# lhn0323/BEVFUSION-3D_object_detection

Hardware: AMD Instinct MI355X
Metric: nuScenes frames/sec (6-cam+LiDAR BEVFusion fwd+bwd) (higher is better)
Workload: dtype bf16; 1 GPU; full: BEVFusion camera+LiDAR (ResNet-50, LSS 6x256x704, hard voxelize 40k pts, sparse encoder, ConvFuser, SECOND/SECONDFPN, TransFusion head + Hungarian targets + focal/L1/gaussian-focal losses) fwd + bwd + clip + AdamW, bf16 autocast, fp32 index paths; global_batch=4, points_per_frame=40000, parallelism=independent frames per rank, execution=eager launches on 2 HIP queues (camera / BEV chain, LiDAR branch), view_transform_conv_dtype=bf16, head_fp32_conv=three bf16 products per multiply, fp32 accumulation (2^-16 relative per product), dense_weight_gradients=one grouped launch per tile shape at the end of the backward pass, backward_pass_thread=caller, trainable_params=37361053

## Files before the change

### bevfusion-3d_object_detection_amd/_lib.py

```python
import ctypes
import os

import torch

_HERE = os.path.dirname(os.path.abspath(__file__))
LIB_PATH = os.path.join(_HERE, "csrc", "libbevfusion_hip.so")

_c_int = ctypes.c_int
_c_vp = ctypes.c_void_p
_c_sz = ctypes.c_size_t

SIGNATURES = {
    "bfhip_abi_version": (_c_int, []),
    "bfhip_last_error": (ctypes.c_char_p, []),
    "bfhip_profile_enable": (None, [_c_int]),
    "bfhip_profile_read": (_c_int, [_c_int, _c_vp, _c_vp, _c_int]),
    "bfhip_bev_pool_fwd": (_c_int, [_c_vp] * 5 + [_c_int] * 7 + [_c_vp, _c_vp]),
    "bfhip_bev_pool_bwd": (_c_int, [_c_vp] * 5 + [_c_int] * 8 + [_c_vp, _c_vp]),
    "bfhip_dynamic_voxelize": (_c_int, [_c_vp, _c_vp, _c_int, _c_int, _c_vp, _c_vp, _c_vp]),
    "bfhip_hard_voxelize_workspace_bytes": (_c_sz, [_c_int, _c_int, _c_int]),
    "bfhip_hard_voxelize": (_c_int, [_c_vp, _c_int, _c_int, _c_vp, _c_vp, _c_vp, _c_vp, _c_vp,
                                     _c_int, _c_int, _c_vp, _c_sz, _c_vp, _c_vp]),
    "bfhip_bev_plan_workspace_bytes": (_c_sz, [ctypes.c_longlong, ctypes.c_longlong]),
    "bfhip_bev_plan": (_c_int, [_c_vp] * 7 + [_c_int] * 4 + [_c_vp] * 3 + [_c_vp] * 11 + [_c_int, _c_vp, _c_sz, _c_vp]),
# ... 77 lines not shown
    "bfhip_conv2d_dgrad_wt": (_c_int, [_c_vp, _c_int, _c_vp, _c_vp, _c_int, _c_vp, _c_int] + [_c_int] * 11 + [_c_vp]),
    "bfhip_conv2d_dgrad_fuses_addend": (_c_int, [_c_int] * 5),
    "bfhip_split_bf16x3": (_c_int, [_c_vp, ctypes.c_longlong, _c_int, _c_vp, _c_int, _c_vp, _c_int, _c_vp]),
    "bfhip_conv2d_wt_segment_bytes": (_c_int, []),
    "bfhip_conv2d_weight_transpose_batched": (_c_int, [_c_vp, _c_int, ctypes.c_longlong, _c_vp]),
    "bfhip_conv2d_launch_choice": (_c_int, [_c_int] * 12 + [_c_vp]),
    "bfhip_conv2d_wgrad_choice": (_c_int, [_c_int] * 10 + [_c_vp]),
    "bfhip_conv2d_wgrad_workspace_bytes": (_c_sz, [_c_int] * 7),
    "bfhip_conv2d_wgrad": (_c_int, [_c_vp, _c_int, _c_vp, _c_int, _c_vp] + [_c_int] * 11 + [_c_vp, _c_sz, _c_vp]),
    "bfhip_conv2d_wgrad_group_table_bytes": (_c_sz, [_c_int]),
    "bfhip_conv2d_wgrad_groupable": (_c_int, [_c_int] * 10),
    "bfhip_conv2d_wgrad_group_plan": (_c_int, [_c_vp, _c_int, _c_int, _c_vp, _c_sz, _c_vp]),
    "bfhip_conv2d_wgrad_group_launch": (_c_int, [_c_vp, _c_vp, _c_vp, _c_sz, _c_vp]),
    "bfhip_bn2d_fwd_partials": (_c_int, [_c_vp] * 4 + [ctypes.c_longlong, _c_int, _c_int, ctypes.c_float, ctypes.c_float, _c_int] +
                                [_c_vp] * 4 + [_c_vp, _c_int, _c_vp, _c_vp]),
    "bfhip_bn2d_fwd_partials_mask": (_c_int, [_c_vp] * 4 + [ctypes.c_longlong, _c_int, _c_int, ctypes.c_float, ctypes.c_float, _c_int] +
                                     [_c_vp] * 4 + [_c_vp, _c_int, _c_vp, _c_vp, _c_vp]),
    "bfhip_bn2d_bwd_mask": (_c_int, [_c_vp] * 5 + [ctypes.c_longlong, _c_int, _c_int] + [_c_vp] * 4 + [_c_vp, _c_sz, _c_vp]),
    "bfhip_adamw_segment_bytes": (_c_int, []),
    "bfhip_adamw_chunk_elems": (_c_int, []),
    "bfhip_adamw_step": (_c_int, [_c_vp, _c_vp, _c_vp, _c_int, _c_vp, _c_vp] + [ctypes.c_float] * 6 + [_c_vp]),
    "bfhip_query_losses": (_c_int, [_c_vp] * 7 + [_c_int] * 6 + [ctypes.c_float, ctypes.c_float] + [_c_vp] * 4),
    "bfhip_swin_attn_supported": (_c_int, [_c_int] * 7),
    "bfhip_swin_attn_parts": (_c_int, [_c_int] * 4),
    "bfhip_swin_attn_fwd": (_c_int, [_c_vp, ctypes.c_longlong, _c_vp] + [_c_int] * 5 + [ctypes.c_float, _c_vp, _c_vp, _c_vp]),
    "bfhip_swin_attn_bwd": (_c_int, [_c_vp, ctypes.c_longlong, _c_vp, _c_vp, _c_vp, _c_vp] + [_c_int] * 5 +
                            [ctypes.c_float, _c_vp, _c_vp, _c_int, _c_vp]),
    "bfhip_layernorm_supported": (_c_int, [ctypes.c_longlong, _c_int, _c_int, _c_int]),
    "bfhip_layernorm_parts": (_c_int, [ctypes.c_longlong, _c_int]),
    "bfhip_layernorm_fwd": (_c_int, [_c_vp, _c_vp, _c_vp, ctypes.c_longlong, _c_vp, _c_vp, ctypes.c_longlong, _c_int, ctypes.c_float] +
                            [_c_int] * 3 + [_c_vp] * 4),
    "bfhip_layernorm_bwd": (_c_int, [_c_vp] * 6 + [ctypes.c_longlong, ctypes.c_longlong] + [_c_int] * 4 + [_c_vp] * 3 + [_c_int] +
                            [_c_vp] * 3),
}

_lib = None


def load():
    global _lib
    if _lib is None:
        if not os.path.exists(LIB_PATH):
            raise RuntimeError(
                "libbevfusion_hip.so not found at %s: build it with "
                "`python -c 'import __graft_entry__ as g; g.build()'` (hipcc, gfx950). "
                "There is no CPU fallback." % LIB_PATH)
        lib = ctypes.CDLL(LIB_PATH)
        for name, (res, args) in SIGNATURES.items():
            fn = getattr(lib, name)
            fn.restype = res
            fn.argtypes = args
        _lib = lib
    return _lib


_torch_ext = False


def torch_ext():
    global _torch_ext
    if _torch_ext is False:
        _torch_ext = None
        path = os.path.join(_HERE, "csrc", "bfhip_torch_ext.so")
        if os.environ.get("BFHIP_TORCH_EXT", "1") == "1" and os.path.exists(path):
            import importlib.util
            load()
# ... 33 lines not shown

def ptr(t):
    return None if t is None else t.data_ptr()


_raw_stream = getattr(torch._C, "_cuda_getCurrentRawStream", None)


def stream_of(t):
    if _raw_stream is not None:
        return _raw_stream(t.device.index if t.device.index is not None else torch.cuda.current_device())
    return ctypes.c_void_p(torch.cuda.current_stream(t.device).cuda_stream)


def host_i32(values):
    return (ctypes.c_int32 * len(values))(*[int(v) for v in values])


def host_f32(values):
    arr = (ctypes.c_float * len(values))(*[float(v) for v in values])
    return arr


def require_cuda(t, name):
    if not t.is_cuda:
        raise RuntimeError("%s must be a CUDA(HIP) tensor; this build has no CPU path" % name)
    if not t.is_contiguous():
        raise RuntimeError("%s must be contiguous" % name)


OPS = dict(bev_pool_fwd=0, bev_pool_bwd=1, hard_voxelize=2, dynamic_voxelize=3, lift_splat_fwd=4, lift_splat_bwd=5,
           spconv_fwd=6, spconv_bwd=7, rulebook=8, bev_aux=9, scatter_fwd=10, scatter_bwd=11, spconv_wgrad=12, raster=13,
           spconv_wgrad_main=14, conv2d_fwd=15, conv2d_dgrad=16, conv2d_wgrad=17, bn2d_fwd=18, bn2d_bwd=19,
           conv2d_pw_fwd=20, conv2d_pw_dgrad=21)


def profile_enable(on=True):
    load().bfhip_profile_enable(int(on))


def profile_read(op, reset=True):
    s = ctypes.c_double(0.0)
    c = ctypes.c_longlong(0)
    check(load().bfhip_profile_read(OPS[op] if isinstance(op, str) else op, ctypes.byref(s), ctypes.byref(c),
                                    1 if reset else 0), "profile_read")
    return s.value, c.value
```

### bevfusion-3d_object_detection_amd/dense_modules.py

```python
import os

import torch
import torch.nn.functional as F
from torch import nn

from . import _lib
from .bn2d import BatchNorm2dAct, BatchNormRows, bn_act
from .conv2d import Conv2d, Conv2dHipWgrad, fp32_island
from .linear_rows import linear_rows
from . import attention as split_attention
from .registry import MODELS


_RESNET_CONV = os.environ.get("BFHIP_RESNET_CONV", "tuned")


def _resnet_conv(cin, cout, k, stride=1, padding=0, bias=False):
    mode = _RESNET_CONV
    if mode == "tuned":
        m = Conv2dHipWgrad(cin, cout, k, stride=stride, padding=padding, bias=bias)
        if stride == 1 and k == 1:
            m.fwd = m.dgrad = "hip"
        elif k == 3:
            m.dgrad = "hip"
            if cin <= 256:
                m.fwd = "hip"
        elif k == 1:
            m.cache_wt = True
        return m
    if k == 1:
        cls = Conv2d if mode == "hip" else (Conv2dHipWgrad if mode in ("hipwgrad", "hip3x3+hipwgrad") else nn.Conv2d)
    else:
        cls = Conv2d if mode in ("hip", "hip3x3", "hip3x3+hipwgrad") else (Conv2dHipWgrad if mode == "hipwgrad" else nn.Conv2d)
    return cls(cin, cout, k, stride=stride, padding=padding, bias=bias)


_Conv3x3 = _Conv1x1 = _resnet_conv
_SHORTCUT_FORK = os.environ.get("BFHIP_SHORTCUT_FORK", "1") == "1"
_HEAD_ROWS = os.environ.get("BFHIP_HEAD_ROWS", "1") == "1"


class _Bottleneck(nn.Module):
    expansion = 4

    def __init__(self, inplanes, planes, stride=1, downsample=None):
        super().__init__()
        self.conv1 = _Conv1x1(inplanes, planes, 1, bias=False)
        self.bn1 = BatchNorm2dAct(planes)
        self.conv2 = _Conv3x3(planes, planes, 3, stride=stride, padding=1, bias=False)
        self.bn2 = BatchNorm2dAct(planes)
        self.conv3 = _Conv1x1(planes, planes * 4, 1, bias=False)
        self.bn3 = BatchNorm2dAct(planes * 4)
        self.relu = nn.ReLU(inplace=True)
        self.downsample = downsample

    def forward(self, x):
        ds = self.downsample
        if ds is None and hasattr(self.conv1, "forward_fork"):
            out, identity = self.conv1.forward_fork(x)
            out = self.bn1(out, relu=True)
        elif (ds is not None and hasattr(self.conv1, "forward_fork") and isinstance(ds[0], Conv2dHipWgrad) and ds[0].stride == (2, 2)
              and ds[0].kernel_size == (1, 1) and ds[0].padding == (0, 0) and _SHORTCUT_FORK and ds[0].training):
            out, x_sub = self.conv1.forward_fork(x, subsample=2)
            out = self.bn1(out, relu=True)
            identity = ds(x) if x_sub is None else ds[1](ds[0].forward_unstrided(x_sub))
        else:
            identity = x if self.downsample is None else self.downsample(x)
            out = self.bn1(self.conv1(x), relu=True)
        out = self.bn2(self.conv2(out), relu=True)
        return self.bn3(self.conv3(out), residual=identity, relu=True)


# ... 297 lines not shown
        self.norms = nn.ModuleList([nn.LayerNorm(d) for _ in range(3)])
        self.self_posembed = PositionEncodingLearned(**pos_encoding_cfg)
        self.cross_posembed = PositionEncodingLearned(**pos_encoding_cfg)

    def forward(self, query, key=None, query_pos=None, key_pos=None):
        qp = self.self_posembed.forward_nlc(query_pos)
        kp = self.cross_posembed.forward_nlc(key_pos)
        q, k = query.transpose(1, 2), key.transpose(1, 2)
        qq = q + qp
        q = self.norms[0](self.self_attn.attend(q, qq, qq, qq))
        kk = k + kp
        q = self.norms[1](self.cross_attn.attend(q, q + qp, kk, kk))
        q = self.norms[2](self.ffn(q))
        return q.transpose(1, 2)


class SeparateHead(nn.Module):
    def __init__(self, in_channels, heads, head_conv=64, final_kernel=1, init_bias=-2.19):
        super().__init__()
        self.heads = heads
        for head, (classes, num_conv) in heads.items():
            layers, c_in = [], in_channels
            for _ in range(num_conv - 1):
                layers.append(ConvModule(c_in, head_conv, final_kernel, padding=final_kernel // 2, dim=1))
                c_in = head_conv
            layers.append(nn.Conv1d(head_conv, classes, final_kernel, padding=final_kernel // 2, bias=True))
            self.add_module(head, nn.Sequential(*layers))
        getattr(self, "heatmap")[-1].bias.data.fill_(init_bias)

    def _pointwise(self):
        return all(isinstance(m, (ConvModule, nn.Conv1d)) and (m.conv if isinstance(m, ConvModule) else m).kernel_size == (1,)
                   and (m.conv if isinstance(m, ConvModule) else m).stride == (1,) for head in self.heads for m in getattr(self, head))

    def forward(self, x):
        if not (_HEAD_ROWS and x.is_cuda and x.dim() == 3 and self._pointwise()):
            return {head: getattr(self, head)(x) for head in self.heads}
        B, C, L = x.shape
        rows = x.transpose(1, 2).reshape(B * L, C)
        if torch.is_autocast_enabled("cuda") and rows.dtype != torch.get_autocast_dtype("cuda"):
            rows = rows.to(torch.get_autocast_dtype("cuda"))
        out = {}
        for head in self.heads:
            h = rows
            for m in getattr(self, head):
                if isinstance(m, ConvModule):
                    h = F.linear(h, m.conv.weight.squeeze(-1), m.conv.bias)
                    if m.bn is not None:
                        h = m.bn(h, relu=m.act)
                    elif m.act:
                        h = F.relu(h)
                else:
                    h = F.linear(h, m.weight.squeeze(-1), m.bias)
            out[head] = h.view(B, L, -1).transpose(1, 2)
        return out


@MODELS.register_module()
class BEVFusionHead(nn.Module):

    def __init__(self, num_proposals=200, auxiliary=True, in_channels=512, hidden_channel=128, num_classes=10,
                 num_decoder_layers=1, decoder_layer=dict(), num_heads=8, nms_kernel_size=3, bn_momentum=0.1,
                 common_heads=dict(center=[2, 2], height=[1, 2], dim=[3, 2], rot=[2, 2], vel=[2, 2]),
                 num_heatmap_convs=2, grid_size=(1440, 1440, 41), out_size_factor=8, train_cfg=None, test_cfg=None,
                 bbox_coder=None,
                 loss_cls=dict(type="mmdet.FocalLoss", use_sigmoid=True, gamma=2.0, alpha=0.25, reduction="mean", loss_weight=1.0),
                 loss_bbox=dict(type="mmdet.L1Loss", reduction="mean", loss_weight=0.25),
                 loss_heatmap=dict(type="mmdet.GaussianFocalLoss", reduction="mean", loss_weight=1.0), **kwargs):
        super().__init__()
        from .head_targets import TransFusionBBoxCoder, _assigner_weights
        self.train_cfg, self.test_cfg = train_cfg, test_cfg
        self.loss_cls_cfg, self.loss_bbox_cfg, self.loss_heatmap_cfg = dict(loss_cls), dict(loss_bbox), dict(loss_heatmap)
# ... 191 lines not shown
```

### include/bevfusion_hip.h

```cpp
#ifndef BEVFUSION_HIP_H_
#define BEVFUSION_HIP_H_

#include <stddef.h>
#include <stdint.h>

#ifdef __cplusplus
extern "C" {
#endif

#define BFHIP_OK 0
#define BFHIP_E_INVALID (-1)
#define BFHIP_E_WORKSPACE (-2)
#define BFHIP_E_LAUNCH (-3)

#define BFHIP_REDUCE_SUM 0
#define BFHIP_REDUCE_MEAN 1
#define BFHIP_REDUCE_MAX 2

#define BFHIP_OP_BEV_POOL_FWD 0
#define BFHIP_OP_BEV_POOL_BWD 1
#define BFHIP_OP_HARD_VOXELIZE 2
#define BFHIP_OP_DYNAMIC_VOXELIZE 3
#define BFHIP_OP_LIFT_SPLAT_FWD 4
#define BFHIP_OP_LIFT_SPLAT_BWD 5
#define BFHIP_OP_SPCONV_FWD 6
#define BFHIP_OP_SPCONV_BWD 7
#define BFHIP_OP_RULEBOOK 8
#define BFHIP_OP_BEV_AUX 9
#define BFHIP_OP_SCATTER_FWD 10
#define BFHIP_OP_SCATTER_BWD 11
#define BFHIP_OP_SPCONV_WGRAD 12
#define BFHIP_OP_RASTER 13
#define BFHIP_OP_SPCONV_WGRAD_MAIN 14
#define BFHIP_OP_CONV2D_FWD 15
#define BFHIP_OP_CONV2D_DGRAD 16
#define BFHIP_OP_CONV2D_WGRAD 17
#define BFHIP_OP_BN2D_FWD 18
#define BFHIP_OP_BN2D_BWD 19
#define BFHIP_OP_CONV2D_PW_FWD 20
#define BFHIP_OP_CONV2D_PW_DGRAD 21
#define BFHIP_OP_COUNT 24

int bfhip_abi_version(void);
const char *bfhip_last_error(void);

void bfhip_profile_enable(int on);
int bfhip_profile_read(int op, double *sum_ms_host, long long *count_host, int reset);

int bfhip_bev_pool_fwd(const float *x, const int32_t *geom, const int32_t *starts,
                       const int32_t *lengths, float *out, int n, int c, int m, int b, int d,
                       int h, int w, const int32_t *m_dev, void *stream);
int bfhip_bev_pool_bwd(const float *out_grad, const int32_t *geom, const int32_t *starts,
                       const int32_t *lengths, float *x_grad, int n, int c, int m, int b, int d,
                       int h, int w, int intervals_cover_all_rows, const int32_t *m_dev,
                       void *stream);

int bfhip_dynamic_voxelize(const float *points, int32_t *coors, int n, int f,
                           const float *voxel_size_host, const float *coors_range_host,
                           void *stream);
size_t bfhip_hard_voxelize_workspace_bytes(int n, int max_points, int max_voxels);
int bfhip_hard_voxelize(const float *points, int n, int f, float *voxels, int32_t *coors,
                        int32_t *num_points_per_voxel, const float *voxel_size_host,
                        const float *coors_range_host, int max_points, int max_voxels,
                        void *workspace, size_t workspace_bytes, int32_t *voxel_num_dev,
                        void *stream);

size_t bfhip_dynamic_scatter_workspace_bytes(int N);
int bfhip_dynamic_scatter_fwd(const float *feats, const int32_t *coors, int N, int C, int reduce_type,
                              float *voxel_feats, int32_t *voxel_coors, int32_t *point2voxel,
                              int32_t *voxel_count, int32_t *counts_dev, void *workspace,
                              size_t workspace_bytes, void *stream);
size_t bfhip_dynamic_scatter_bwd_workspace_bytes(int M, int C);
int bfhip_dynamic_scatter_bwd(float *grad_feats, const float *grad_voxel_feats, const float *feats,
// ... 194 lines not shown
                            float *stats, void *y, const float *partial, int nblk, const int32_t *m_dev, void *stream);
int bfhip_bn2d_fwd_partials_mask(const void *x, const void *residual, const float *gamma, const float *beta, long long M, int C,
                                 int dtype, float eps, float momentum, int relu, float *running_mean, float *running_var,
                                 float *stats, void *y, const float *partial, int nblk, const int32_t *m_dev,
                                 unsigned char *relu_mask, void *stream);
int bfhip_bn2d_bwd_mask(const void *dy, const void *x, const unsigned char *relu_mask, const float *stats, const float *gamma,
                        long long M, int C, int dtype, void *dx, void *dres, float *dgb, const int32_t *m_dev, void *workspace,
                        size_t workspace_bytes, void *stream);

int bfhip_adamw_segment_bytes(void);
int bfhip_adamw_chunk_elems(void);
int bfhip_adamw_step(const void *segs_dev, const int64_t *grad_ptrs_dev, const int32_t *chunks_dev, int n_chunks,
                     float *partial_dev, float *scalars_dev, float lr, float beta1, float beta2, float eps,
                     float weight_decay, float max_norm, void *stream);

int bfhip_swin_attn_supported(int B, int Hp, int Wp, int heads, int window, int head_dim, int shift);
int bfhip_swin_attn_parts(int B, int Hp, int Wp, int heads);
int bfhip_swin_attn_fwd(const void *qkv, long long qkv_pitch, const float *bias, int B, int Hp, int Wp, int heads, int shift,
                        float scale, void *out, float *lse, void *stream);
int bfhip_swin_attn_bwd(const void *qkv, long long qkv_pitch, const float *bias, const void *out, const void *dout,
                        const float *lse, int B, int Hp, int Wp, int heads, int shift, float scale, void *dqkv,
                        float *dbias_partial, int parts, void *stream);

int bfhip_layernorm_supported(long long M, int C, int x_dtype, int y_dtype);
int bfhip_layernorm_parts(long long M, int C);
int bfhip_layernorm_fwd(const void *x, const void *branch, const float *scale, long long rows_per_sample, const float *gamma,
                        const float *beta, long long M, int C, float eps, int x_dtype, int branch_dtype, int y_dtype, void *s,
                        void *y, float *mean_rstd, void *stream);
int bfhip_layernorm_bwd(const void *s, const float *mean_rstd, const float *gamma, const void *dy, const void *dsum,
                        const float *scale, long long rows_per_sample, long long M, int C, int x_dtype, int branch_dtype,
                        int y_dtype, void *dx, void *dbranch, float *partial, int parts, float *dgamma, float *dbeta,
                        void *stream);

#ifdef __cplusplus
}
#endif
#endif
```

Measured before the change: 152.6 frames/s.

## Fuse TransFusion prediction heads into single multi-head HIP kernels for fwd and bwd

```diff
diff --git a/bevfusion-3d_object_detection_amd/_lib.py b/bevfusion-3d_object_detection_amd/_lib.py
--- a/bevfusion-3d_object_detection_amd/_lib.py
+++ b/bevfusion-3d_object_detection_amd/_lib.py
@@ -133,6 +133,10 @@
                             [_c_int] * 3 + [_c_vp] * 4),
     "bfhip_layernorm_bwd": (_c_int, [_c_vp] * 6 + [ctypes.c_longlong, ctypes.c_longlong] + [_c_int] * 4 + [_c_vp] * 3 + [_c_int] +
                             [_c_vp] * 3),
+    "bfhip_pred_heads_supported": (_c_int, [_c_int] * 5),
+    "bfhip_pred_heads_workspace_bytes": (_c_sz, [_c_int] * 4),
+    "bfhip_pred_heads_fwd": (_c_int, [_c_vp] + [_c_int] * 6 + [_c_vp] * 5),
+    "bfhip_pred_heads_bwd": (_c_int, [_c_vp] + [_c_int] * 7 + [_c_vp] * 5 + [_c_sz, _c_vp]),
 }
 
 _lib = None
@@ -232,7 +236,7 @@
 OPS = dict(bev_pool_fwd=0, bev_pool_bwd=1, hard_voxelize=2, dynamic_voxelize=3, lift_splat_fwd=4, lift_splat_bwd=5,
            spconv_fwd=6, spconv_bwd=7, rulebook=8, bev_aux=9, scatter_fwd=10, scatter_bwd=11, spconv_wgrad=12, raster=13,
            spconv_wgrad_main=14, conv2d_fwd=15, conv2d_dgrad=16, conv2d_wgrad=17, bn2d_fwd=18, bn2d_bwd=19,
-           conv2d_pw_fwd=20, conv2d_pw_dgrad=21)
+           conv2d_pw_fwd=20, conv2d_pw_dgrad=21, pred_heads_fwd=22, pred_heads_bwd=23)
 
 
 def profile_enable(on=True):
diff --git a/bevfusion-3d_object_detection_amd/csrc/pred_heads.hip b/bevfusion-3d_object_detection_amd/csrc/pred_heads.hip
--- /dev/null
+++ b/bevfusion-3d_object_detection_amd/csrc/pred_heads.hip
@@ -0,0 +1,648 @@
+#include "common.h"
+
+namespace bfhip {
+namespace {
+
+typedef unsigned short bf16_t;
+typedef short s16x4 __attribute__((ext_vector_type(4)));
+typedef float f32x4 __attribute__((ext_vector_type(4)));
+#define MFMA16(a, b, c) __builtin_amdgcn_mfma_f32_16x16x16bf16_1k(a, b, c, 0, 0, 0)
+
+constexpr int kMaxHeads = 8, kMaxR = 1024, kMaxCin = 128, kMaxHidden = 64, kMaxK = 16;
+constexpr int kThreads = 1024, kWaves = kThreads / 64;
+constexpr int kPad = 4;
+constexpr int kScratchFloats = 4096;
+constexpr int kSmallFloats = 8 * kMaxHidden;
+
+__device__ __forceinline__ float bf2f(bf16_t v) { return __uint_as_float((unsigned)v << 16); }
+__device__ __forceinline__ bf16_t f2bf(float f) {
+  unsigned u = __float_as_uint(f);
+  if ((u & 0x7fffffffu) > 0x7f800000u) return (bf16_t)((u >> 16) | 0x40u);
+  return (bf16_t)((u + 0x7fffu + ((u >> 16) & 1u)) >> 16);
+}
+template <bool F32>
+__device__ __forceinline__ bf16_t ldw(const void *p, unsigned i) {
+  return F32 ? f2bf(((const float *)p)[i]) : ((const bf16_t *)p)[i];
+}
+template <bool F32>
+__device__ __forceinline__ float ldwf(const void *p, unsigned i) {
+  return F32 ? ((const float *)p)[i] : bf2f(((const bf16_t *)p)[i]);
+}
+__device__ __forceinline__ s16x4 zero4() { s16x4 r = {0, 0, 0, 0}; return r; }
+__device__ __forceinline__ s16x4 unpack4(uint2 u) {
+  s16x4 r;
+  r[0] = (short)(u.x & 0xffffu); r[1] = (short)(u.x >> 16); r[2] = (short)(u.y & 0xffffu); r[3] = (short)(u.y >> 16);
+  return r;
+}
+template <bool XF32>
+__device__ __forceinline__ s16x4 ldx4(const void *X, unsigned off) {
+  if (XF32) {
+    const float4 v = *(const float4 *)((const float *)X + off);
+    s16x4 r;
+    r[0] = (short)f2bf(v.x); r[1] = (short)f2bf(v.y); r[2] = (short)f2bf(v.z); r[3] = (short)f2bf(v.w);
+    return r;
+  }
+  return unpack4(*(const uint2 *)((const bf16_t *)X + off));
+}
+template <bool F32>
+__device__ __forceinline__ s16x4 ldw4(const void *W, unsigned off) { return ldx4<F32>(W, off); }
+template <bool XF32>
+__device__ __forceinline__ short ldx1(const void *X, unsigned off) {
+  return XF32 ? (short)f2bf(((const float *)X)[off]) : (short)((const bf16_t *)X)[off];
+}
+
+struct HeadFwd {
+  const void *w1, *b1;
+  const float *gamma, *beta;
+  float *running_mean, *running_var;
+  const void *w2, *b2;
+  bf16_t *out, *h1;
+  float *stats;
+  int k;
+  float eps, momentum;
+};
+struct FwdArgs { HeadFwd h[kMaxHeads]; };
+
+struct HeadBwd {
+  const void *w1, *w2;
+  const bf16_t *h1;
+  const float *stats;
+  const bf16_t *dout;
+  int sb, sl, sk;
+  float *dw1, *db1, *dgamma, *dbeta, *dw2, *db2;
+  int k;
+};
+struct BwdArgs { HeadBwd h[kMaxHeads]; };
+
+inline size_t lds_bytes(int R, int hidden) {
+  const int Rp = (R + 15) & ~15;
+  return (size_t)Rp * (hidden + kPad) * 2 + (size_t)(kScratchFloats + kSmallFloats) * 4;
+}
+
+template <bool XF32, bool WF32>
+__global__ __launch_bounds__(kThreads) void pred_heads_fwd_kernel(const void *__restrict__ X, int R, int Cin, int Hd, FwdArgs args) {
+  extern __shared__ __align__(16) unsigned char smem[];
+  const HeadFwd &hd = args.h[blockIdx.x];
+  const int Rp = (R + 15) & ~15, ldh = Hd + kPad, ntiles = Rp >> 4, nts = Hd >> 4, nks = Cin >> 4;
+  bf16_t *Hs = (bf16_t *)smem;
+  float *scratch = (float *)(smem + (size_t)Rp * ldh * 2);
+  float *sA = scratch + kScratchFloats, *sB = sA + kMaxHidden;
+  const int tid = threadIdx.x, w = tid >> 6, lane = tid & 63, ln = lane & 15, lg = lane >> 4;
+
+  {
+    s16x4 bw[kMaxHidden / 16][kMaxCin / 16];
+    float b1v[kMaxHidden / 16];
+#pragma unroll
+    for (int nt = 0; nt < kMaxHidden / 16; ++nt) {
+      b1v[nt] = (nt < nts && hd.b1) ? ldwf<WF32>(hd.b1, nt * 16 + ln) : 0.f;
+#pragma unroll
+      for (int ks = 0; ks < kMaxCin / 16; ++ks)
+        bw[nt][ks] = (nt < nts && ks < nks) ? ldw4<WF32>(hd.w1, (unsigned)(nt * 16 + ln) * Cin + ks * 16 + lg * 4) : zero4();
+    }
+    for (int t = w; t < ntiles; t += kWaves) {
+      const int r = t * 16 + ln;
+      s16x4 a[kMaxCin / 16];
+#pragma unroll
+      for (int ks = 0; ks < kMaxCin / 16; ++ks)
+        a[ks] = (ks < nks && r < R) ? ldx4<XF32>(X, (unsigned)r * Cin + ks * 16 + lg * 4) : zero4();
+#pragma unroll
+      for (int nt = 0; nt < kMaxHidden / 16; ++nt) {
+        if (nt < nts) {
+          f32x4 acc = {0.f, 0.f, 0.f, 0.f};
+#pragma unroll
+          for (int ks = 0; ks < kMaxCin / 16; ++ks)
+            if (ks < nks) acc = MFMA16(a[ks], bw[nt][ks], acc);
+          const int c = nt * 16 + ln;
+#pragma unroll
+          for (int j = 0; j < 4; ++j) {
+            const int row = t * 16 + lg * 4 + j;
+            const bf16_t v = f2bf(acc[j] + b1v[nt]);
+            Hs[row * ldh + c] = row < R ? v : (bf16_t)0;
+            if (row < R) hd.h1[(unsigned)row * Hd + c] = v;
+          }
+        }
+      }
+    }
+  }
+  __syncthreads();
+
+  {
+    const int G = kThreads / Hd, c = tid % Hd, g = tid / Hd;
+    if (g < G) {
+      float s = 0.f, s2 = 0.f;
+      for (int r = g; r < R; r += G) {
+        const float v = bf2f(Hs[r * ldh + c]);
+        s += v;
+        s2 += v * v;
+      }
+      scratch[g * Hd + c] = s;
+      scratch[kScratchFloats / 2 + g * Hd + c] = s2;
+    }
+    __syncthreads();
+    if (tid < Hd) {
+      double s = 0.0, s2 = 0.0;
+      for (int g2 = 0; g2 < G; ++g2) {
+        s += (double)scratch[g2 * Hd + tid];
+        s2 += (double)scratch[kScratchFloats / 2 + g2 * Hd + tid];
+      }
+      const double mean = s / (double)R;
+      double var = s2 / (double)R - mean * mean;
+      if (var < 0.0) var = 0.0;
+      const float invstd = (float)(1.0 / sqrt(var + (double)hd.eps));
+      const float a = hd.gamma[tid] * invstd;
+      const float b = hd.beta[tid] - (float)mean * a;
+      hd.stats[tid] = (float)mean;
+      hd.stats[Hd + tid] = invstd;
+      hd.stats[2 * Hd + tid] = a;
+      hd.stats[3 * Hd + tid] = b;
+      sA[tid] = a;
+      sB[tid] = b;
+      if (hd.running_mean) {
+        const double unbiased = R > 1 ? var * (double)R / (double)(R - 1) : var;
+        hd.running_mean[tid] = (float)((1.0 - hd.momentum) * hd.running_mean[tid] + hd.momentum * mean);
+        hd.running_var[tid] = (float)((1.0 - hd.momentum) * hd.running_var[tid] + hd.momentum * unbiased);
+      }
+    }
+    __syncthreads();
+  }
+
+  {
+    const int k = hd.k;
+    s16x4 w2f[kMaxHidden / 16];
+    float av[kMaxHidden / 16][4], bv[kMaxHidden / 16][4];
+#pragma unroll
+    for (int ks = 0; ks < kMaxHidden / 16; ++ks) {
+      w2f[ks] = (ks < nts && ln < k) ? ldw4<WF32>(hd.w2, (unsigned)ln * Hd + ks * 16 + lg * 4) : zero4();
+#pragma unroll
+      for (int j = 0; j < 4; ++j) {
+        av[ks][j] = 0.f; bv[ks][j] = 0.f;
+        if (ks < nts) {
+          const int c = ks * 16 + lg * 4 + j;
+          av[ks][j] = sA[c]; bv[ks][j] = sB[c];
+        }
+      }
+    }
+    const float b2v = ln < k ? ldwf<WF32>(hd.b2, ln) : 0.f;
+    for (int t = w; t < ntiles; t += kWaves) {
+      f32x4 acc = {0.f, 0.f, 0.f, 0.f};
+#pragma unroll
+      for (int ks = 0; ks < kMaxHidden / 16; ++ks) {
+        if (ks < nts) {
+          const s16x4 h = unpack4(*(const uint2 *)(Hs + (t * 16 + ln) * ldh + ks * 16 + lg * 4));
+          s16x4 y;
+#pragma unroll
+          for (int j = 0; j < 4; ++j) {
+            const float z = bf2f((bf16_t)h[j]) * av[ks][j] + bv[ks][j];
+            y[j] = (short)f2bf(z > 0.f ? z : 0.f);
+          }
+          acc = MFMA16(y, w2f[ks], acc);
+        }
+      }
+#pragma unroll
+      for (int j = 0; j < 4; ++j) {
+        const int row = t * 16 + lg * 4 + j;
+        if (row < R && ln < k) hd.out[(unsigned)row * k + ln] = f2bf(acc[j] + b2v);
+      }
+    }
+  }
+}
+
+__device__ __forceinline__ short ld_dout(const HeadBwd &hd, int r, int kk, int R, int L) {
+  const bf16_t *base = hd.dout ? hd.dout : hd.h1;
+  const bool ok = hd.dout && r < R && kk < hd.k;
+  const int b = r / L, l = r - b * L;
+  const bf16_t v = base[ok ? (unsigned)(b * hd.sb + l * hd.sl + kk * hd.sk) : 0u];
+  return ok ? (short)v : (short)0;
+}
+
+template <bool XF32, bool WF32>
+__global__ __launch_bounds__(kThreads) void pred_heads_bwd_kernel(const void *__restrict__ X, int R, int L, int Cin, int Hd,
+                                                                   float *__restrict__ dx_part, float *dw1_parts, BwdArgs args) {
+  extern __shared__ __align__(16) unsigned char smem[];
+  const HeadBwd &hd = args.h[blockIdx.x];
+  const int Rp = (R + 15) & ~15, ldh = Hd + kPad, ntiles = Rp >> 4, nts = Hd >> 4, nn = Cin >> 4, k = hd.k;
+  bf16_t *Hs = (bf16_t *)smem;
+  float *scratch = (float *)(smem + (size_t)Rp * ldh * 2);
+  float *sMean = scratch + kScratchFloats, *sInv = sMean + kMaxHidden, *sA = sInv + kMaxHidden, *sB = sA + kMaxHidden;
+  float *sC1 = sB + kMaxHidden, *sC2 = sC1 + kMaxHidden, *sC3 = sC2 + kMaxHidden;
+  const int tid = threadIdx.x, w = tid >> 6, lane = tid & 63, ln = lane & 15, lg = lane >> 4;
+
+  {
+    const int q = Hd >> 2, n = Rp * q;
+    for (int i0 = tid; i0 < n; i0 += 4 * kThreads) {
+      uint2 v[4];
+#pragma unroll
+      for (int u = 0; u < 4; ++u) {
+        const int idx = i0 + u * kThreads, r = idx / q, c4 = (idx - r * q) * 4;
+        v[u] = make_uint2(0u, 0u);
+        if (idx < n && r < R) v[u] = *(const uint2 *)(hd.h1 + (unsigned)r * Hd + c4);
+      }
+#pragma unroll
+      for (int u = 0; u < 4; ++u) {
+        const int idx = i0 + u * kThreads, r = idx / q, c4 = (idx - r * q) * 4;
+        if (idx < n) *(uint2 *)(Hs + r * ldh + c4) = v[u];
+      }
+    }
+    if (tid < Hd) {
+      sMean[tid] = hd.stats[tid];
+      sInv[tid] = hd.stats[Hd + tid];
+      sA[tid] = hd.stats[2 * Hd + tid];
+      sB[tid] = hd.stats[3 * Hd + tid];
+    }
+  }
+  __syncthreads();
+
+  float ca[kMaxHidden / 16], cb[kMaxHidden / 16], cm[kMaxHidden / 16];
+  s16x4 w2b[kMaxHidden / 16];
+#pragma unroll
+  for (int nt = 0; nt < kMaxHidden / 16; ++nt) {
+    ca[nt] = cb[nt] = cm[nt] = 0.f;
+    w2b[nt] = zero4();
+    if (nt < nts) {
+      const int c = nt * 16 + ln;
+      ca[nt] = sA[c]; cb[nt] = sB[c]; cm[nt] = sMean[c];
+#pragma unroll
+      for (int j = 0; j < 4; ++j) {
+        const int kk = lg * 4 + j;
+        const short v = (short)ldw<WF32>(hd.w2, (size_t)(kk < k ? kk : 0) * Hd + c);
+        w2b[nt][j] = kk < k ? v : (short)0;
+      }
+    }
+  }
+  constexpr int kOwn = kMaxR / 16 / kWaves;
+  s16x4 da[kOwn];
+#pragma unroll
+  for (int u = 0; u < kOwn; ++u)
+#pragma unroll
+    for (int j = 0; j < 4; ++j) da[u][j] = ld_dout(hd, (w + u * kWaves) * 16 + ln, lg * 4 + j, R, L);
+
+  {
+    float s0[kMaxHidden / 16], s1[kMaxHidden / 16], ds[4] = {0.f, 0.f, 0.f, 0.f};
+#pragma unroll
+    for (int nt = 0; nt < kMaxHidden / 16; ++nt) s0[nt] = s1[nt] = 0.f;
+#pragma unroll
+    for (int u = 0; u < kOwn; ++u) {
+      const int t = w + u * kWaves;
+      if (t >= ntiles) continue;
+      const s16x4 a = da[u];
+#pragma unroll
+      for (int j = 0; j < 4; ++j) ds[j] += bf2f((bf16_t)a[j]);
+#pragma unroll
+      for (int nt = 0; nt < kMaxHidden / 16; ++nt) {
+        if (nt < nts) {
+          const f32x4 acc = MFMA16(a, w2b[nt], ((f32x4){0.f, 0.f, 0.f, 0.f}));
+#pragma unroll
+          for (int j = 0; j < 4; ++j) {
+            const float h = bf2f(Hs[(t * 16 + lg * 4 + j) * ldh + nt * 16 + ln]);
+            const float g = (h * ca[nt] + cb[nt] > 0.f) ? bf2f(f2bf(acc[j])) : 0.f;
+            s0[nt] += g;
+            s1[nt] += g * (h - cm[nt]);
+          }
+        }
+      }
+    }
+#pragma unroll
+    for (int nt = 0; nt < kMaxHidden / 16; ++nt) {
+      s0[nt] += __shfl_xor(s0[nt], 16); s0[nt] += __shfl_xor(s0[nt], 32);
+      s1[nt] += __shfl_xor(s1[nt], 16); s1[nt] += __shfl_xor(s1[nt], 32);
+      if (nt < nts && lg == 0) {
+        scratch[(w * 2 + 0) * kMaxHidden + nt * 16 + ln] = s0[nt];
+        scratch[(w * 2 + 1) * kMaxHidden + nt * 16 + ln] = s1[nt];
+      }
+    }
+#pragma unroll
+    for (int j = 0; j < 4; ++j) {
+      float v = ds[j];
+      v += __shfl_xor(v, 1); v += __shfl_xor(v, 2); v += __shfl_xor(v, 4); v += __shfl_xor(v, 8);
+      if (ln == 0) scratch[2 * kWaves * kMaxHidden + w * 16 + lg * 4 + j] = v;
+    }
+  }
+  __syncthreads();
+  if (tid < Hd) {
+    double s = 0.0, s2 = 0.0;
+    for (int w2 = 0; w2 < kWaves; ++w2) {
+      s += (double)scratch[(w2 * 2 + 0) * kMaxHidden + tid];
+      s2 += (double)scratch[(w2 * 2 + 1) * kMaxHidden + tid];
+    }
+    const float mean = sMean[tid], invstd = sInv[tid], a = sA[tid];
+    const float dbeta = (float)s, dgamma = (float)(s2 * (double)invstd);
+    hd.dgamma[tid] = dgamma;
+    hd.dbeta[tid] = dbeta;
+    const float invM = (float)(1.0 / (double)R);
+    const float c2 = -a * invstd * dgamma * invM;
+    sC1[tid] = a;
+    sC2[tid] = c2;
+    sC3[tid] = -a * dbeta * invM - c2 * mean;
+  } else if (tid >= kMaxHidden && tid < kMaxHidden + k) {
+    const int kk = tid - kMaxHidden;
+    double s = 0.0;
+    for (int w2 = 0; w2 < kWaves; ++w2) s += (double)scratch[2 * kWaves * kMaxHidden + w2 * 16 + kk];
+    hd.db2[kk] = (float)s;
+  }
+  __syncthreads();
+
+  {
+    constexpr int nq = 4;
+    const int nt = w % nts, kq = w / nts;
+    if (kq < nq) {
+      const float a_ = sA[nt * 16 + ln], b_ = sB[nt * 16 + ln];
+      f32x4 acc = {0.f, 0.f, 0.f, 0.f};
+      for (int t0 = kq; t0 < ntiles; t0 += 4 * nq) {
+        s16x4 a[4];
+#pragma unroll
+        for (int u = 0; u < 4; ++u)
+#pragma unroll
+          for (int j = 0; j < 4; ++j) a[u][j] = ld_dout(hd, (t0 + u * nq) * 16 + lg * 4 + j, ln, R, L);
+#pragma unroll
+        for (int u = 0; u < 4; ++u) {
+          const int t = t0 + u * nq;
+          if (t < ntiles) {
+            s16x4 y;
+#pragma unroll
+            for (int j = 0; j < 4; ++j) {
+              const float z = bf2f(Hs[(t * 16 + lg * 4 + j) * ldh + nt * 16 + ln]) * a_ + b_;
+              y[j] = (short)f2bf(z > 0.f ? z : 0.f);
+            }
+            acc = MFMA16(a[u], y, acc);
+          }
+        }
+      }
+#pragma unroll
+      for (int j = 0; j < 4; ++j) scratch[(kq * 16 + lg * 4 + j) * kMaxHidden + nt * 16 + ln] = acc[j];
+    }
+    __syncthreads();
+    if (tid < k * Hd) {
+      const int kk = tid / Hd, c = tid - kk * Hd;
+      float s = 0.f;
+      for (int q2 = 0; q2 < nq; ++q2) s += scratch[(q2 * 16 + kk) * kMaxHidden + c];
+      hd.dw2[kk * Hd + c] = s;
+    }
+  }
+
+  {
+    float c1[kMaxHidden / 16], c2[kMaxHidden / 16], c3[kMaxHidden / 16];
+#pragma unroll
+    for (int nt = 0; nt < kMaxHidden / 16; ++nt) {
+      c1[nt] = c2[nt] = c3[nt] = 0.f;
+      if (nt < nts) { c1[nt] = sC1[nt * 16 + ln]; c2[nt] = sC2[nt * 16 + ln]; c3[nt] = sC3[nt * 16 + ln]; }
+    }
+#pragma unroll
+    for (int u = 0; u < kOwn; ++u) {
+      const int t = w + u * kWaves;
+      if (t >= ntiles) continue;
+      const s16x4 a = da[u];
+#pragma unroll
+      for (int nt = 0; nt < kMaxHidden / 16; ++nt) {
+        if (nt < nts) {
+          const f32x4 acc = MFMA16(a, w2b[nt], ((f32x4){0.f, 0.f, 0.f, 0.f}));
+#pragma unroll
+          for (int j = 0; j < 4; ++j) {
+            const int row = t * 16 + lg * 4 + j;
+            bf16_t *p = Hs + row * ldh + nt * 16 + ln;
+            const float h = bf2f(*p);
+            const float g = (h * ca[nt] + cb[nt] > 0.f) ? bf2f(f2bf(acc[j])) : 0.f;
+            *p = row < R ? f2bf(c1[nt] * g + c2[nt] * h + c3[nt]) : (bf16_t)0;
+          }
+        }
+      }
+    }
+  }
+  __syncthreads();
+
+  if (hd.db1) {
+    const int G = kThreads / Hd, c = tid % Hd, g = tid / Hd;
+    if (g < G) {
+      float s = 0.f;
+      for (int r = g; r < R; r += G) s += bf2f(Hs[r * ldh + c]);
+      scratch[g * Hd + c] = s;
+    }
+    __syncthreads();
+    if (tid < Hd) {
+      double s = 0.0;
+      for (int g2 = 0; g2 < G; ++g2) s += (double)scratch[g2 * Hd + tid];
+      hd.db1[tid] = (float)s;
+    }
+  }
+
+  const int w1_ni = w % nn, w1_kh = w / nn;
+  float *dw1_part = dw1_parts + (size_t)blockIdx.x * Hd * Cin;
+  f32x4 w1acc[kMaxHidden / 16];
+#pragma unroll
+  for (int u = 0; u < kMaxHidden / 16; ++u) w1acc[u] = (f32x4){0.f, 0.f, 0.f, 0.f};
+  if (w1_kh < 2) {
+    const int i = w1_ni * 16 + ln;
+    constexpr int TB = 4;
+    for (int t0 = w1_kh; t0 < ntiles; t0 += 2 * TB) {
+      s16x4 xb[TB];
+#pragma unroll
+      for (int v = 0; v < TB; ++v)
+#pragma unroll
+        for (int j = 0; j < 4; ++j) {
+          const int r = (t0 + 2 * v) * 16 + lg * 4 + j;
+          const short x = ldx1<XF32>(X, (unsigned)(r < R ? r : 0) * Cin + i);
+          xb[v][j] = r < R ? x : (short)0;
+        }
+#pragma unroll
+      for (int v = 0; v < TB; ++v) {
+        const int t = t0 + 2 * v;
+        if (t < ntiles) {
+#pragma unroll
+          for (int u = 0; u < kMaxHidden / 16; ++u) {
+            if (u < nts) {
+              s16x4 a;
+#pragma unroll
+              for (int j = 0; j < 4; ++j) a[j] = (short)Hs[(t * 16 + lg * 4 + j) * ldh + u * 16 + ln];
+              w1acc[u] = MFMA16(a, xb[v], w1acc[u]);
+            }
+          }
+        }
+      }
+    }
+    if (w1_kh == 1) {
+#pragma unroll
+      for (int u = 0; u < kMaxHidden / 16; ++u) {
+        if (u < nts) {
+#pragma unroll
+          for (int j = 0; j < 4; ++j) dw1_part[(unsigned)(u * 16 + lg * 4 + j) * Cin + i] = w1acc[u][j];
+        }
+      }
+    }
+  }
+
+  {
+    const int ng = kWaves / nn, ni = w % nn, rg = w / nn;
+    if (rg < ng) {
+      const int i = ni * 16 + ln;
+      s16x4 w1b[kMaxHidden / 16];
+#pragma unroll
+      for (int ks = 0; ks < kMaxHidden / 16; ++ks) {
+        w1b[ks] = zero4();
+        if (ks < nts) {
+#pragma unroll
+          for (int j = 0; j < 4; ++j) w1b[ks][j] = (short)ldw<WF32>(hd.w1, (unsigned)(ks * 16 + lg * 4 + j) * Cin + i);
+        }
+      }
+      float *part = dx_part + (size_t)blockIdx.x * R * Cin;
+      for (int t = rg; t < ntiles; t += ng) {
+        f32x4 acc = {0.f, 0.f, 0.f, 0.f};
+#pragma unroll
+        for (int ks = 0; ks < kMaxHidden / 16; ++ks) {
+          if (ks < nts) {
+            const s16x4 a = unpack4(*(const uint2 *)(Hs + (t * 16 + ln) * ldh + ks * 16 + lg * 4));
+            acc = MFMA16(a, w1b[ks], acc);
+          }
+        }
+#pragma unroll
+        for (int j = 0; j < 4; ++j) {
+          const int row = t * 16 + lg * 4 + j;
+          if (row < R) part[(unsigned)row * Cin + i] = acc[j];
+        }
+      }
+    }
+  }
+
+  __syncthreads();
+  if (w1_kh == 0) {
+    const int i = w1_ni * 16 + ln;
+#pragma unroll
+    for (int u = 0; u < kMaxHidden / 16; ++u) {
+      if (u < nts) {
+#pragma unroll
+        for (int j = 0; j < 4; ++j) {
+          const unsigned o = (unsigned)(u * 16 + lg * 4 + j) * Cin + i;
+          hd.dw1[o] = w1acc[u][j] + dw1_part[o];
+        }
+      }
+    }
+  }
+}
+
+template <bool XF32>
+__global__ __launch_bounds__(256) void pred_heads_dx_kernel(const float *__restrict__ part, int n_heads, int n4, void *__restrict__ dx) {
+  const int idx = blockIdx.x * 256 + threadIdx.x;
+  if (idx >= n4) return;
+  float4 s = ((const float4 *)part)[idx];
+  for (int h = 1; h < n_heads; ++h) {
+    const float4 v = ((const float4 *)part)[(size_t)h * n4 + idx];
+    s.x += v.x; s.y += v.y; s.z += v.z; s.w += v.w;
+  }
+  if (XF32) {
+    ((float4 *)dx)[idx] = s;
+  } else {
+    uint2 o;
+    o.x = (unsigned)f2bf(s.x) | ((unsigned)f2bf(s.y) << 16);
+    o.y = (unsigned)f2bf(s.z) | ((unsigned)f2bf(s.w) << 16);
+    ((uint2 *)dx)[idx] = o;
+  }
+}
+
+bool shape_ok(int R, int Cin, int hidden, int n_heads, int max_k) {
+  return R >= 2 && R <= kMaxR && Cin >= 16 && Cin <= kMaxCin && Cin % 16 == 0 && hidden >= 16 && hidden <= kMaxHidden &&
+         hidden % 16 == 0 && n_heads >= 1 && n_heads <= kMaxHeads && max_k >= 1 && max_k <= kMaxK;
+}
+
+constexpr int kLdsLimit = 160 * 1024;
+
+}
+}
+
+using namespace bfhip;
+
+BFHIP_EXPORT int bfhip_pred_heads_supported(int R, int Cin, int hidden, int n_heads, int max_k) {
+  return shape_ok(R, Cin, hidden, n_heads, max_k) && lds_bytes(R, hidden) <= (size_t)kLdsLimit ? 1 : 0;
+}
+
+BFHIP_EXPORT size_t bfhip_pred_heads_workspace_bytes(int R, int Cin, int hidden, int n_heads) {
+  if (!shape_ok(R, Cin, hidden, n_heads, 1)) return 0;
+  return align_up((size_t)n_heads * ((size_t)R * Cin + (size_t)hidden * Cin) * sizeof(float), 256);
+}
+
+BFHIP_EXPORT int bfhip_pred_heads_fwd(const void *x, int x_dtype, int w_dtype, int R, int Cin, int hidden, int n_heads,
+                                      const int *head_k, const float *head_eps, const float *head_momentum,
+                                      const void *const *head_ptrs, void *stream) {
+  BFHIP_REQUIRE(x && head_k && head_eps && head_momentum && head_ptrs, "pred_heads_fwd: null argument");
+  BFHIP_REQUIRE((x_dtype == 0 || x_dtype == 1) && (w_dtype == 0 || w_dtype == 1), "pred_heads_fwd: dtypes must be 0 (f32) or 1 (bf16)");
+  int max_k = 0;
+  for (int h = 0; h < n_heads && h < kMaxHeads; ++h) max_k = head_k[h] > max_k ? head_k[h] : max_k;
+  BFHIP_REQUIRE(bfhip_pred_heads_supported(R, Cin, hidden, n_heads, max_k), "pred_heads_fwd: unsupported shape R=%d Cin=%d hidden=%d heads=%d k<=%d",
+                R, Cin, hidden, n_heads, max_k);
+  BFHIP_REQUIRE(((uintptr_t)x & 15) == 0, "pred_heads_fwd: x must be 16-byte aligned");
+  FwdArgs args{};
+  for (int h = 0; h < n_heads; ++h) {
+    const void *const *p = head_ptrs + (size_t)h * BFHIP_PRED_HEADS_FWD_PTRS;
+    BFHIP_REQUIRE(head_k[h] >= 1, "pred_heads_fwd: head %d has k = %d", h, head_k[h]);
+    BFHIP_REQUIRE(p[0] && p[2] && p[3] && p[6] && p[7] && p[8] && p[9] && p[10], "pred_heads_fwd: head %d has a null pointer", h);
+    BFHIP_REQUIRE((p[4] == nullptr) == (p[5] == nullptr), "pred_heads_fwd: head %d: running_mean and running_var go together", h);
+    BFHIP_REQUIRE(((uintptr_t)p[9] & 7) == 0, "pred_heads_fwd: head %d: h1 must be 8-byte aligned", h);
+    BFHIP_REQUIRE((((uintptr_t)p[0] | (uintptr_t)p[6]) & 15) == 0, "pred_heads_fwd: head %d: W1 and W2 must be 16-byte aligned", h);
+    HeadFwd &a = args.h[h];
+    a.w1 = p[0]; a.b1 = p[1]; a.gamma = (const float *)p[2]; a.beta = (const float *)p[3];
+    a.running_mean = (float *)p[4]; a.running_var = (float *)p[5];
+    a.w2 = p[6]; a.b2 = p[7]; a.out = (bf16_t *)p[8]; a.h1 = (bf16_t *)p[9]; a.stats = (float *)p[10];
+    a.k = head_k[h]; a.eps = head_eps[h]; a.momentum = head_momentum[h];
+  }
+  hipStream_t s = (hipStream_t)stream;
+  const size_t lds = lds_bytes(R, hidden);
+  ProfScope ps;
+  prof_begin(BFHIP_OP_PRED_HEADS_FWD, s, &ps);
+#define BFHIP_PH_FWD(XF, WF) \
+  launch_big_lds<pred_heads_fwd_kernel<XF, WF>>(kLdsLimit, dim3((unsigned)n_heads), dim3(kThreads), lds, s, x, R, Cin, hidden, args)
+  if (x_dtype == 0) { if (w_dtype == 0) BFHIP_PH_FWD(true, true); else BFHIP_PH_FWD(true, false); }
+  else { if (w_dtype == 0) BFHIP_PH_FWD(false, true); else BFHIP_PH_FWD(false, false); }
+#undef BFHIP_PH_FWD
+  prof_end(&ps);
+  return check_launch("pred_heads_fwd");
+}
+
+BFHIP_EXPORT int bfhip_pred_heads_bwd(const void *x, int x_dtype, int w_dtype, int R, int rows_per_batch, int Cin, int hidden,
+                                      int n_heads, const int *head_k, const void *const *head_ptrs,
+                                      const long long *dout_strides, void *dx, void *workspace, size_t workspace_bytes,
+                                      void *stream) {
+  BFHIP_REQUIRE(x && head_k && head_ptrs && dout_strides && dx, "pred_heads_bwd: null argument");
+  BFHIP_REQUIRE((x_dtype == 0 || x_dtype == 1) && (w_dtype == 0 || w_dtype == 1), "pred_heads_bwd: dtypes must be 0 (f32) or 1 (bf16)");
+  int max_k = 0;
+  for (int h = 0; h < n_heads && h < kMaxHeads; ++h) max_k = head_k[h] > max_k ? head_k[h] : max_k;
+  BFHIP_REQUIRE(bfhip_pred_heads_supported(R, Cin, hidden, n_heads, max_k), "pred_heads_bwd: unsupported shape R=%d Cin=%d hidden=%d heads=%d k<=%d",
+                R, Cin, hidden, n_heads, max_k);
+  BFHIP_REQUIRE(rows_per_batch >= 1 && R % rows_per_batch == 0, "pred_heads_bwd: R = %d is no multiple of rows_per_batch = %d", R, rows_per_batch);
+  BFHIP_REQUIRE((((uintptr_t)x | (uintptr_t)dx | (uintptr_t)workspace) & 15) == 0, "pred_heads_bwd: x, dx and workspace must be 16-byte aligned");
+  if (!workspace || workspace_bytes < bfhip_pred_heads_workspace_bytes(R, Cin, hidden, n_heads)) {
+    set_error("pred_heads_bwd: workspace too small");
+    return BFHIP_E_WORKSPACE;
+  }
+  BwdArgs args{};
+  for (int h = 0; h < n_heads; ++h) {
+    const void *const *p = head_ptrs + (size_t)h * BFHIP_PRED_HEADS_BWD_PTRS;
+    const long long *st = dout_strides + (size_t)h * 3;
+    BFHIP_REQUIRE(head_k[h] >= 1, "pred_heads_bwd: head %d has k = %d", h, head_k[h]);
+    BFHIP_REQUIRE(p[0] && p[1] && p[2] && p[3] && p[5] && p[7] && p[8] && p[9] && p[10], "pred_heads_bwd: head %d has a null pointer", h);
+    BFHIP_REQUIRE(((uintptr_t)p[2] & 7) == 0, "pred_heads_bwd: head %d: h1 must be 8-byte aligned", h);
+    BFHIP_REQUIRE(!p[4] || (st[0] >= 0 && st[1] >= 0 && st[2] >= 0), "pred_heads_bwd: head %d: negative dOut stride", h);
+    BFHIP_REQUIRE(!p[4] || (R / rows_per_batch - 1) * st[0] + (rows_per_batch - 1) * st[1] + (head_k[h] - 1) * st[2] < (1LL << 31),
+                  "pred_heads_bwd: head %d: dOut spans 2^31 elements or more", h);
+    HeadBwd &a = args.h[h];
+    a.w1 = p[0]; a.w2 = p[1]; a.h1 = (const bf16_t *)p[2]; a.stats = (const float *)p[3]; a.dout = (const bf16_t *)p[4];
+    a.sb = (int)st[0]; a.sl = (int)st[1]; a.sk = (int)st[2];
+    a.dw1 = (float *)p[5]; a.db1 = (float *)p[6]; a.dgamma = (float *)p[7]; a.dbeta = (float *)p[8];
+    a.dw2 = (float *)p[9]; a.db2 = (float *)p[10];
+    a.k = head_k[h];
+  }
+  hipStream_t s = (hipStream_t)stream;
+  const size_t lds = lds_bytes(R, hidden);
+  const int n4 = R * Cin / 4;
+  ProfScope ps;
+  prof_begin(BFHIP_OP_PRED_HEADS_BWD, s, &ps);
+#define BFHIP_PH_BWD(XF, WF)                                                                                                      \
+  launch_big_lds<pred_heads_bwd_kernel<XF, WF>>(kLdsLimit, dim3((unsigned)n_heads), dim3(kThreads), lds, s, x, R, rows_per_batch, Cin, \
+                                                hidden, (float *)workspace, (float *)workspace + (size_t)n_heads * R * Cin, args)
+  if (x_dtype == 0) {
+    if (w_dtype == 0) BFHIP_PH_BWD(true, true); else BFHIP_PH_BWD(true, false);
+    hipLaunchKernelGGL(pred_heads_dx_kernel<true>, dim3(ceil_div(n4, 256)), dim3(256), 0, s, (const float *)workspace, n_heads, n4, dx);
+  } else {
+    if (w_dtype == 0) BFHIP_PH_BWD(false, true); else BFHIP_PH_BWD(false, false);
+    hipLaunchKernelGGL(pred_heads_dx_kernel<false>, dim3(ceil_div(n4, 256)), dim3(256), 0, s, (const float *)workspace, n_heads, n4, dx);
+  }
+#undef BFHIP_PH_BWD
+  prof_end(&ps);
+  return check_launch("pred_heads_bwd");
+}
diff --git a/bevfusion-3d_object_detection_amd/dense_modules.py b/bevfusion-3d_object_detection_amd/dense_modules.py
--- a/bevfusion-3d_object_detection_amd/dense_modules.py
+++ b/bevfusion-3d_object_detection_amd/dense_modules.py
@@ -9,6 +9,8 @@
 from .conv2d import Conv2d, Conv2dHipWgrad, fp32_island
 from .linear_rows import linear_rows
 from . import attention as split_attention
+from . import bn2d as _bn2d
+from . import pred_heads as _pred_heads
 from .registry import MODELS
 
 
@@ -38,6 +40,7 @@
 _Conv3x3 = _Conv1x1 = _resnet_conv
 _SHORTCUT_FORK = os.environ.get("BFHIP_SHORTCUT_FORK", "1") == "1"
 _HEAD_ROWS = os.environ.get("BFHIP_HEAD_ROWS", "1") == "1"
+_PRED_HEADS = os.environ.get("BFHIP_PRED_HEADS", "1") == "1"
 
 
 class _Bottleneck(nn.Module):
@@ -401,11 +404,43 @@
         return all(isinstance(m, (ConvModule, nn.Conv1d)) and (m.conv if isinstance(m, ConvModule) else m).kernel_size == (1,)
                    and (m.conv if isinstance(m, ConvModule) else m).stride == (1,) for head in self.heads for m in getattr(self, head))
 
+    def _conv_bn_relu_conv(self):
+        stacks = []
+        for head in self.heads:
+            seq = getattr(self, head)
+            if not (len(seq) == 2 and isinstance(seq[0], ConvModule) and isinstance(seq[0].bn, BatchNormRows) and seq[0].act
+                    and isinstance(seq[0].conv, nn.Conv1d) and isinstance(seq[1], nn.Conv1d)
+                    and seq[0].conv.groups == 1 and seq[1].groups == 1):
+                return None
+            stacks.append((seq[0].conv, seq[0].bn, seq[1]))
+        return stacks
+
+    def _fusable_stacks(self, rows):
+        stacks = self._conv_bn_relu_conv_cache
+        if stacks is None:
+            stacks = self._conv_bn_relu_conv_cache = self._conv_bn_relu_conv() or ()
+        if not stacks:
+            return None
+        key = (rows.dtype, rows.shape[0], torch.is_autocast_enabled("cuda") and torch.get_autocast_dtype("cuda"),
+               stacks[0][0].weight.dtype, stacks[0][0].weight.device) + tuple(bn.training for _, bn, _ in stacks)
+        if key != self._fusable_key:
+            self._fusable_key, self._fusable = key, _pred_heads.fusable(rows, stacks)
+        return stacks if self._fusable else None
+
+    _conv_bn_relu_conv_cache = None
+    _fusable_key = None
+    _fusable = False
+
     def forward(self, x):
         if not (_HEAD_ROWS and x.is_cuda and x.dim() == 3 and self._pointwise()):
             return {head: getattr(self, head)(x) for head in self.heads}
         B, C, L = x.shape
         rows = x.transpose(1, 2).reshape(B * L, C)
+        if _PRED_HEADS and self.training and _bn2d.FUSED_BN2D and rows.is_contiguous() and rows.data_ptr() % 16 == 0:
+            stacks = self._fusable_stacks(rows)
+            if stacks is not None:
+                outs = _pred_heads.pred_heads(rows, B, L, stacks)
+                return {head: o.transpose(1, 2) for head, o in zip(self.heads, outs)}
         if torch.is_autocast_enabled("cuda") and rows.dtype != torch.get_autocast_dtype("cuda"):
             rows = rows.to(torch.get_autocast_dtype("cuda"))
         out = {}
diff --git a/bevfusion-3d_object_detection_amd/pred_heads.py b/bevfusion-3d_object_detection_amd/pred_heads.py
--- /dev/null
+++ b/bevfusion-3d_object_detection_amd/pred_heads.py
@@ -0,0 +1,127 @@
+import ctypes
+
+import torch
+
+from . import _lib
+
+_DT = {torch.float32: 0, torch.bfloat16: 1}
+_FWD_PTRS = _BWD_PTRS = 11
+_SUPPORTED = {}
+
+
+def supported(R, Cin, hidden, n_heads, max_k):
+    key = (R, Cin, hidden, n_heads, max_k)
+    ok = _SUPPORTED.get(key)
+    if ok is None:
+        ok = _SUPPORTED[key] = bool(_lib.load().bfhip_pred_heads_supported(R, Cin, hidden, n_heads, max_k))
+    return ok
+
+
+def _ptr(t):
+    return None if t is None else t.data_ptr()
+
+
+class _PredHeadsFunction(torch.autograd.Function):
+
+    @staticmethod
+    def forward(ctx, rows, B, L, bns, *params):
+        n = len(bns)
+        R, Cin = rows.shape
+        hidden = params[0].shape[0]
+        dev = rows.device
+        ks = [params[6 * i + 4].shape[0] for i in range(n)]
+        outs = [torch.empty((B, L, k), dtype=torch.bfloat16, device=dev) for k in ks]
+        h1 = torch.empty((n, R, hidden), dtype=torch.bfloat16, device=dev)
+        stats = torch.empty((n, 4 * hidden), dtype=torch.float32, device=dev)
+        ptrs = (ctypes.c_void_p * (n * _FWD_PTRS))()
+        for i, bn in enumerate(bns):
+            w1, b1, gamma, beta, w2, b2 = params[6 * i:6 * i + 6]
+            ptrs[i * _FWD_PTRS:(i + 1) * _FWD_PTRS] = [w1.data_ptr(), _ptr(b1), gamma.data_ptr(), beta.data_ptr(),
+                                                      bn.running_mean.data_ptr(), bn.running_var.data_ptr(), w2.data_ptr(),
+                                                      b2.data_ptr(), outs[i].data_ptr(), h1[i].data_ptr(), stats[i].data_ptr()]
+        _lib.call("bfhip_pred_heads_fwd", rows.data_ptr(), _DT[rows.dtype], _DT[params[0].dtype], R, Cin, hidden, n,
+                  _lib.host_i32(ks), _lib.host_f32([bn.eps for bn in bns]), _lib.host_f32([bn.momentum for bn in bns]), ptrs,
+                  _lib.stream_of(rows))
+        ctx.save_for_backward(rows, h1, stats, *params)
+        ctx.dims = (n, R, L, Cin, hidden, ks)
+        return tuple(outs)
+
+    @staticmethod
+    @torch.autograd.function.once_differentiable
+    def backward(ctx, *douts):
+        rows, h1, stats, *params = ctx.saved_tensors
+        n, R, L, Cin, hidden, ks = ctx.dims
+        dev = rows.device
+        low = params[0].dtype
+        conv_sizes = []
+        for i in range(n):
+            w1, b1, _, _, w2, b2 = params[6 * i:6 * i + 6]
+            conv_sizes.append((w1.numel(), 0 if b1 is None else b1.numel(), w2.numel(), b2.numel()))
+        n_conv = sum(sum(s) for s in conv_sizes)
+        n_conv_pad = -(-n_conv // 4) * 4
+        buf = torch.empty(n_conv_pad + n * 2 * hidden, dtype=torch.float32, device=dev)
+        base, esz = buf.data_ptr(), 4
+        ptrs = (ctypes.c_void_p * (n * _BWD_PTRS))()
+        strides = (ctypes.c_longlong * (n * 3))()
+        keep, off = [], 0
+        for i in range(n):
+            w1, b1, _, _, w2, _ = params[6 * i:6 * i + 6]
+            s_w1, s_b1, s_w2, s_b2 = conv_sizes[i]
+            o_w1, o_b1, o_w2, o_b2 = off, off + s_w1, off + s_w1 + s_b1, off + s_w1 + s_b1 + s_w2
+            off = o_b2 + s_b2
+            o_g = n_conv_pad + i * 2 * hidden
+            d = douts[i]
+            if d is not None:
+                if d.dtype != torch.bfloat16:
+                    d = d.to(torch.bfloat16)
+                keep.append(d)
+                strides[3 * i:3 * i + 3] = list(d.stride())
+            ptrs[i * _BWD_PTRS:(i + 1) * _BWD_PTRS] = [w1.data_ptr(), w2.data_ptr(), h1[i].data_ptr(), stats[i].data_ptr(), _ptr(d),
+                                                      base + o_w1 * esz, (base + o_b1 * esz) if s_b1 else None, base + o_g * esz,
+                                                      base + (o_g + hidden) * esz, base + o_w2 * esz, base + o_b2 * esz]
+        dx = torch.empty_like(rows)
+        nbytes = _lib.call_size("bfhip_pred_heads_workspace_bytes", R, Cin, hidden, n)
+        ws = torch.empty(nbytes, dtype=torch.uint8, device=dev)
+        _lib.call("bfhip_pred_heads_bwd", rows.data_ptr(), _DT[rows.dtype], _DT[low], R, L, Cin, hidden, n, _lib.host_i32(ks), ptrs,
+                  strides, dx.data_ptr(), ws.data_ptr(), ws.numel(), _lib.stream_of(rows))
+        conv = buf[:n_conv] if low == torch.float32 else buf[:n_conv].to(low)
+        c_parts = iter(conv.split([x for s in conv_sizes for x in s if x]))
+        g_parts = iter(buf[n_conv_pad:].split(hidden))
+        grads = []
+        for i in range(n):
+            w1, b1, _, _, w2, _ = params[6 * i:6 * i + 6]
+            grads += [next(c_parts).view(w1.shape), None if b1 is None else next(c_parts), next(g_parts), next(g_parts),
+                      next(c_parts).view(w2.shape), next(c_parts)]
+        return (dx, None, None, None) + tuple(grads)
+
+
+def pred_heads(rows, B, L, stacks):
+    params, bns = [], []
+    for conv1, bn, conv2 in stacks:
+        params += [conv1.weight, conv1.bias, bn.weight, bn.bias, conv2.weight, conv2.bias]
+        bns.append(bn)
+        bn._pending_batches += 1
+    return _PredHeadsFunction.apply(rows, B, L, bns, *params)
+
+
+def fusable(rows, stacks):
+    autocast = torch.is_autocast_enabled("cuda") and torch.get_autocast_dtype("cuda") == torch.bfloat16
+    if not (rows.dtype == torch.bfloat16 or (autocast and rows.dtype == torch.float32)):
+        return False
+    conv1, bn, conv2 = stacks[0]
+    low, hidden, cin = conv1.weight.dtype, conv1.out_channels, conv1.in_channels
+    if not (low == torch.bfloat16 or (autocast and low == torch.float32)):
+        return False
+    has_b1 = conv1.bias is not None
+    for conv1, bn, conv2 in stacks:
+        if (conv1.out_channels != hidden or conv1.in_channels != cin or conv2.in_channels != hidden or conv2.bias is None
+                or (conv1.bias is not None) != has_b1 or not bn.affine or not bn.track_running_stats or bn.momentum is None
+                or not bn.training or bn.num_features != hidden):
+            return False
+        for p in (conv1.weight, conv1.bias, conv2.weight, conv2.bias):
+            if p is not None and not (p.dtype == low and p.is_cuda and p.is_contiguous() and p.data_ptr() % 16 == 0):
+                return False
+        for p in (bn.weight, bn.bias, bn.running_mean, bn.running_var):
+            if not (p.dtype == torch.float32 and p.is_cuda and p.is_contiguous()):
+                return False
+    return supported(rows.shape[0], cin, hidden, len(stacks), max(c2.out_channels for _, _, c2 in stacks))
diff --git a/include/bevfusion_hip.h b/include/bevfusion_hip.h
--- a/include/bevfusion_hip.h
+++ b/include/bevfusion_hip.h
@@ -39,6 +39,8 @@
 #define BFHIP_OP_BN2D_BWD 19
 #define BFHIP_OP_CONV2D_PW_FWD 20
 #define BFHIP_OP_CONV2D_PW_DGRAD 21
+#define BFHIP_OP_PRED_HEADS_FWD 22
+#define BFHIP_OP_PRED_HEADS_BWD 23
 #define BFHIP_OP_COUNT 24
 
 int bfhip_abi_version(void);
@@ -299,6 +301,16 @@
                         int y_dtype, void *dx, void *dbranch, float *partial, int parts, float *dgamma, float *dbeta,
                         void *stream);
 
+#define BFHIP_PRED_HEADS_FWD_PTRS 11
+#define BFHIP_PRED_HEADS_BWD_PTRS 11
+int bfhip_pred_heads_supported(int R, int Cin, int hidden, int n_heads, int max_k);
+size_t bfhip_pred_heads_workspace_bytes(int R, int Cin, int hidden, int n_heads);
+int bfhip_pred_heads_fwd(const void *x, int x_dtype, int w_dtype, int R, int Cin, int hidden, int n_heads, const int *head_k,
+                         const float *head_eps, const float *head_momentum, const void *const *head_ptrs, void *stream);
+int bfhip_pred_heads_bwd(const void *x, int x_dtype, int w_dtype, int R, int rows_per_batch, int Cin, int hidden, int n_heads,
+                         const int *head_k, const void *const *head_ptrs, const long long *dout_strides, void *dx,
+                         void *workspace, size_t workspace_bytes, void *stream);
+
 #ifdef __cplusplus
 }
 #endif
```

Measured after the change: 154.4 frames/s (median of 6 runs). No clear change (+1.2%).
